# SiftScience/kafka-assigner

Hardware: NVIDIA H100
Metric: partition-replica assignments/sec (higher is better)
Workload: dtype int32

## Files before the change

kafka_assigner_b200/csrc/kassign.cu:

```cuda
#include "kassign_stage.cuh"
#include "kassign_order.cuh"
#include "kassign_json.cuh"
#include "kassign_score.cuh"
#include "kassign_waves.cuh"
#include "kassign_waves_json.cuh"

#include <algorithm>
#include <climits>
#include <cmath>
#include <cstdio>
#include <cstdlib>
#include <cstring>
#include <map>
#include <new>
#include <string>
#include <unordered_map>
#include <vector>

#include "../../include/kassign.h"

namespace {

constexpr int KA_SM_COUNT_FALLBACK = 132;
constexpr size_t KA_SMEM_BUDGET = 200 * 1024;
constexpr uint32_t KA_LUT_SMEM_MAX_RANGE = 32768;
constexpr uint32_t KA_LUT_GLOBAL_MAX_RANGE = 1u << 25;

struct DevBuf {
    void* p = nullptr;
    size_t cap = 0;
    cudaError_t reserve(size_t bytes) {
        if (bytes <= cap) return cudaSuccess;
        if (p) cudaFree(p);
        p = nullptr;
        cap = 0;
        size_t want = bytes + bytes / 8 + 256;
        cudaError_t e = cudaMalloc(&p, want);
        if (e == cudaSuccess) cap = want;
        return e;
    }
    void release() {
        if (p) cudaFree(p);
        p = nullptr;
        cap = 0;
    }
    template <typename T> T* as() const { return reinterpret_cast<T*>(p); }
};

constexpr int KA_MAX_BLOCKS = 8;
constexpr int KA_MAX_CHAIN_BLOCKS = 8;
constexpr int KA_MAX_CHAIN_EVENTS = 64;
constexpr int KA_MAX_JSON_FRAGS = 256;
constexpr int KA_MAX_CANDIDATES = 128;
static_assert(KA_MAX_CANDIDATES <= KA_JSON_MAX_SEGS, "a fleet's documents are built in one segmented JSON pass");
constexpr int64_t KA_JSON_FRAG_ROWS = 1 << 18;

struct HostPinned {
    int err_topic;
    int spin_flag;
    int4 tstatus;
};

struct Plan {
    int a_blob_bytes;
    int a_warps, a_load_bytes, a_slab_bytes, a_cnt_bytes, a_load_kind;
    int a_levels;
    int lv_owner_bytes, lv_last_bytes, lv_p_bytes;
    size_t a_smem;
    int rec_kind, rec_bytes;
    int b_gctr;
    int b_ring_log2;
    int b_threads;
    size_t b_smem;
};

struct StageDesc {
    int topic_base = 0, T = 0;
    int64_t Q = 0;
    const int32_t* d_hash = nullptr;
    const int64_t* d_part_off = nullptr;
    const int64_t* d_rep_off = nullptr;
    int P = 0, RF = 0;
    const int32_t* d_cur = nullptr;
    int desired_rf = -1, S = 1, Pmax = 0;
    int64_t capmax = 0;
    int64_t q0 = 0;
    int blk = 0;
    Plan pl;
};

struct RunScratch {
    DevBuf rec, perm, ntl, lend, loff, lvl_end, tstatus, flags;
    cudaError_t reserve(size_t rec_bytes, size_t q, size_t T, size_t nloff, bool levels, size_t nflags) {
        const struct { DevBuf* b; size_t bytes; } want[] = {
            {&rec, rec_bytes}, {&perm, levels ? q * 2 : 0}, {&lend, levels ? q * 4 : 0}, {&lvl_end, levels ? q * 4 : 0},
            {&ntl, levels ? T * 4 : 0}, {&loff, levels ? nloff * 4 : 0}, {&tstatus, T * sizeof(int4)}, {&flags, nflags * 4},
        };
        for (const auto& w : want)
            if (cudaError_t e = w.b->reserve(w.bytes)) return e;
        return cudaSuccess;
    }
    void release() {
        for (DevBuf* b : {&rec, &perm, &ntl, &lend, &loff, &lvl_end, &tstatus, &flags}) b->release();
    }
};

}

struct ka_ctx {
    int device = 0;
    int sm_count = KA_SM_COUNT_FALLBACK;
    cudaStream_t stream = nullptr;
    cudaStream_t aux = nullptr;
    cudaStream_t sb1 = nullptr;
    cudaStream_t sj = nullptr;
    KaBrokers br{};
    std::vector<int32_t> broker_id;
    DevBuf d_blob, d_glut, d_broker_id, d_ctr8;
    std::unordered_map<int32_t, std::vector<int32_t>> parked;
    int64_t launches = 0;
    DevBuf d_hash, d_part_off, d_rep_off, d_cur, d_out, d_out_len;
    RunScratch run;
    DevBuf d_json, d_names, d_name_off, d_part_id, d_json_rowlen, d_json_blocksum, d_json_state;
    DevBuf d_json_seg;
    DevBuf d_batch_tab, d_batch_ctr;
    RunScratch batch_run;
    DevBuf d_score_w, d_score_sum, d_score_brk, d_score_off;
    DevBuf d_wv_nrecv, d_wv_wave, d_wv_tmp, d_wv_rec, d_wv_cnt, d_wv_state, d_wv_log, d_wv_sum, d_wv_meta;
    DevBuf d_wv_send, d_wv_slog, d_wv_ssum;
    DevBuf d_wv_perm, d_wv_hist, d_wv_doc;
    HostPinned* h_pin = nullptr;
    unsigned long long* h_frag = nullptr;
    cudaEvent_t ev[6] = {};
    cudaEvent_t ev_pipe[KA_MAX_BLOCKS][5] = {};
    cudaEvent_t ev_chain[KA_MAX_CHAIN_EVENTS][4] = {};
    cudaEvent_t ev_in = nullptr, ev_stage[KA_MAX_BLOCKS] = {}, ev_chain_in = nullptr, ev_b1[KA_MAX_CHAIN_EVENTS] = {};
    cudaEvent_t ev_json_in[KA_MAX_JSON_FRAGS] = {}, ev_json_scan[KA_MAX_JSON_FRAGS] = {}, ev_out_done = nullptr;
    bool timing = false;
    float last_ms[8] = {};
    bool ev_valid = false;
    int last_stages = 1;
    int chain_used = 0;
    bool slot_timed[2] = {false, false};
    int32_t order_plan[8] = {};
    int32_t stage_plan[8] = {};
    bool staged = false;
    StageDesc staged_block;
    int topic_base = 0;
    bool last_was_staged = false;
    cudaStream_t last_stream = nullptr;
    bool pending_status = false;
    ka_status last{};
};

namespace {

#define KA_CUDA(call)                                                                              \
    do {                                                                                           \
        cudaError_t _e = (call);                                                                   \
        if (_e != cudaSuccess) {                                                                   \
            std::fprintf(stderr, "[kassign] CUDA error %s at %s:%d: %s\n", cudaGetErrorName(_e), __FILE__, __LINE__, \
                         cudaGetErrorString(_e));                                                  \
            return KA_ERR_CUDA;                                                                    \
        }                                                                                          \
    } while (0)

int set_status(ka_status* st, int code, int topic = -1, int part = -1, int a = 0, int b = 0) {
    if (st) {
        st->code = code;
        st->topic_index = topic;
        st->partition = part;
        st->a = a;
        st->b = b;
    }
    return code;
}

int failed(ka_status* st, int rc) {
    if (st && st->code != rc) set_status(st, rc);
    return rc;
}

inline size_t align16(size_t v) { return (v + 15) & ~size_t(15); }

template <typename F>
void for_each_event(ka_ctx* c, F f) {
    const struct { cudaEvent_t* e; size_t n; bool timed; } pools[] = {
        {c->ev, sizeof(c->ev) / sizeof(cudaEvent_t), true},
        {&c->ev_pipe[0][0], sizeof(c->ev_pipe) / sizeof(cudaEvent_t), true},
        {&c->ev_chain[0][0], sizeof(c->ev_chain) / sizeof(cudaEvent_t), true},
        {&c->ev_in, 1, false},
        {c->ev_stage, KA_MAX_BLOCKS, false},
        {&c->ev_chain_in, 1, false},
        {c->ev_b1, KA_MAX_CHAIN_EVENTS, false},
        {c->ev_json_in, KA_MAX_JSON_FRAGS, false},
        {c->ev_json_scan, KA_MAX_JSON_FRAGS, false},
        {&c->ev_out_done, 1, false},
    };
    for (const auto& p : pools)
        for (size_t i = 0; i < p.n; ++i) f(p.e[i], p.timed);
}

int park_counters(ka_ctx* c) {
    if (c->br.N == 0 || !c->d_ctr8.p) return KA_OK;
    std::vector<int32_t> h((size_t)c->br.N * KA_MAX_SLOTS);
    KA_CUDA(cudaMemcpy(h.data(), c->d_ctr8.p, h.size() * 4, cudaMemcpyDeviceToHost));
    for (int i = 0; i < c->br.N; ++i) {
        const int32_t* row = h.data() + (size_t)i * KA_MAX_SLOTS;
        bool nz = false;
        for (int r = 0; r < KA_MAX_SLOTS; ++r) nz |= row[r] != 0;
        if (nz) c->parked[c->broker_id[i]] = std::vector<int32_t>(row, row + KA_MAX_SLOTS);
        else c->parked.erase(c->broker_id[i]);
    }
    return KA_OK;
}

int check_brokers(int N, const int32_t* broker_id, const int32_t* broker_rack) {
    if (N < 0 || (N > 0 && (!broker_id || !broker_rack))) return KA_ERR_BAD_ARG;
    if (N > 65535) return KA_ERR_LIMIT;
    for (int i = 0; i < N; ++i) {
        if (i > 0 && broker_id[i] <= broker_id[i - 1]) return KA_ERR_BAD_ARG;
        if (broker_rack[i] < 0 || broker_rack[i] >= 65535) return KA_ERR_BAD_ARG;
    }
    return KA_OK;
}

struct BrokerTable {
    int lut_mode = KA_LUT_SMEM, min_id = 0, lut_off = 0;
    uint32_t range = 0;
    std::vector<uint16_t> blob, glut;
    int blob_bytes() const { return (int)(blob.size() * 2); }
    KaBrokers device(int N, const uint16_t* d_blob, const uint16_t* d_glut, const int32_t* d_broker_id) const {
        return KaBrokers{N, lut_mode, lut_off, blob_bytes(), min_id, range, d_blob, d_glut, d_broker_id};
    }
};

BrokerTable broker_table(int N, const int32_t* broker_id, const int32_t* broker_rack) {
    BrokerTable t;
    t.min_id = N > 0 ? broker_id[0] : 0;
    const uint64_t range64 = N > 0 ? (uint64_t)((int64_t)broker_id[N - 1] - (int64_t)broker_id[0]) + 1 : 0;
    const size_t npad = align16((size_t)std::max(N, 1) * 2) / 2;
    std::vector<uint16_t> rackc(std::max(N, 1), 0);
    {
        std::unordered_map<int32_t, int> seen;
        for (int i = 0; i < N; ++i) {
            auto it = seen.find(broker_rack[i]);
            if (it == seen.end()) it = seen.emplace(broker_rack[i], (int)seen.size()).first;
            rackc[i] = (uint16_t)it->second;
        }
    }
    size_t lut_elems = 0;
    if (range64 <= KA_LUT_SMEM_MAX_RANGE) {
        t.lut_mode = KA_LUT_SMEM;
        t.range = (uint32_t)range64;
        lut_elems = align16((size_t)std::max<uint64_t>(range64, 1) * 2) / 2;
    } else if (range64 <= KA_LUT_GLOBAL_MAX_RANGE) {
        t.lut_mode = KA_LUT_GLOBAL;
        t.range = (uint32_t)range64;
        t.glut.assign((size_t)range64, (uint16_t)KA_DEAD);
        for (int i = 0; i < N; ++i) t.glut[(size_t)((int64_t)broker_id[i] - t.min_id)] = (uint16_t)i;
    } else {
        t.lut_mode = KA_LUT_BSEARCH;
        t.range = 0;
    }
    t.lut_off = (int)npad;
    t.blob.assign(npad + lut_elems, (uint16_t)KA_DEAD);
    for (int i = 0; i < N; ++i) {
        t.blob[i] = rackc[i];
        if (t.lut_mode == KA_LUT_SMEM) t.blob[npad + (size_t)((int64_t)broker_id[i] - t.min_id)] = (uint16_t)i;
    }
    return t;
}

constexpr size_t KA_ORDER_SMEM_BUDGET = 226 * 1024;

int make_plan(int N, int blob_bytes, int64_t Q, int S, int Pmax, int64_t capmax, bool ragged, Plan& pl, ka_status* st) {
    if (Q >= (int64_t)1 << 31) return set_status(st, KA_ERR_LIMIT, -1, -1, INT_MAX, 0);
    pl.a_blob_bytes = blob_bytes;
    pl.a_load_kind = capmax <= 255 ? 0 : 1;
    const int lsz = pl.a_load_kind == 0 ? 1 : 2;
    pl.a_load_bytes = (int)align16((size_t)std::max(N, 1) * lsz);
    pl.a_slab_bytes = (int)align16((size_t)std::max(Pmax, 1) * S * 2);
    pl.a_cnt_bytes = (int)align16((size_t)std::max(Pmax, 1));
    pl.a_levels = (capmax > 1 || ragged) ? 1 : 0;
    if (pl.a_levels && Pmax > 32767) return set_status(st, KA_ERR_LIMIT, -1, -1, Pmax, N);
    pl.lv_owner_bytes = pl.a_levels ? (int)align16((size_t)std::max(N, 1) * 4) : 0;
    pl.lv_last_bytes = pl.a_levels ? (int)align16((size_t)std::max(N, 1) * 2) : 0;
    pl.lv_p_bytes = pl.a_levels ? (int)align16((size_t)(std::max(Pmax, 1) + 2) * 2) : 0;
    const size_t per_warp = (size_t)pl.a_load_bytes + pl.a_slab_bytes + pl.a_cnt_bytes + pl.lv_owner_bytes + pl.lv_last_bytes +
                            2 * (size_t)pl.lv_p_bytes;
    const size_t shared = 16 + (size_t)blob_bytes;
    if (shared + per_warp > KA_SMEM_BUDGET) return set_status(st, KA_ERR_LIMIT, -1, -1, Pmax, N);
    pl.a_warps = (int)std::min<size_t>(16, (KA_SMEM_BUDGET - shared) / per_warp);
    pl.a_smem = shared + per_warp * pl.a_warps;
    pl.rec_kind = S <= 3 ? 3 : (S == 4 ? 4 : 8);
    pl.rec_bytes = pl.rec_kind == 3 ? 16 : 32;
    const int cw = pl.rec_kind == 8 ? 8 : 4;
    const int max_nt = pl.rec_kind == 3 ? 1024 : (pl.rec_kind == 4 ? 512 : 256);
    const size_t ctr_bytes = pl.rec_kind == 3 ? (size_t)(std::max(N, 1) + 1) * 4 : (size_t)std::max(N, 1) * cw * 4;
    const int lg_max = pl.rec_kind == 3 ? 10 : 9, lg_min = 7;
    auto ring_bytes = [&](int l) { return ((size_t)KA_RING_STAGES << l) * pl.rec_bytes + 256; };
    int lg = lg_max;
    pl.b_gctr = 0;
    while (lg > lg_min && ctr_bytes + ring_bytes(lg) > KA_ORDER_SMEM_BUDGET) --lg;
    if (ctr_bytes + ring_bytes(lg) > KA_ORDER_SMEM_BUDGET) {
        pl.b_gctr = 1;
        lg = lg_max;
    }
    if (const char* e = std::getenv("KA_ORDER_GLOBAL_CTR")) pl.b_gctr = pl.b_gctr || std::atoi(e);
    pl.b_ring_log2 = lg;
    pl.b_smem = ring_bytes(lg) + (pl.b_gctr ? 0 : ctr_bytes);
    int64_t width = pl.a_levels ? std::min<int64_t>(Pmax, std::max<int64_t>(1, N / std::max(S, 1) / 2)) : Pmax;
    const int64_t cuts = (std::max<int64_t>(width, 1) + max_nt - 1) / max_nt;
    width = (std::max<int64_t>(width, 1) + cuts - 1) / cuts;
    int nt = (int)std::min<int64_t>(max_nt, ((width + 31) / 32) * 32);
    if (const char* e = std::getenv("KA_ORDER_THREADS")) nt = std::atoi(e);
    nt = std::max(32, std::min(max_nt, (nt / 32) * 32));
    nt = std::min(nt, (KA_RING_STAGES - 1) << lg);
    pl.b_threads = nt;
    return KA_OK;
}

template <typename K>
cudaError_t allow_smem(K kernel, size_t bytes) {
    return cudaFuncSetAttribute(kernel, cudaFuncAttributeMaxDynamicSharedMemorySize, (int)bytes);
}

struct Shape {
    int T = 0, P = 0, RF = 0, desired_rf = -1, S = 1;
    const int32_t* d_hash = nullptr;
    const int32_t* d_cur = nullptr;
    const int64_t* d_part_off = nullptr;
    const int64_t* d_rep_off = nullptr;
    int64_t Q = 0, R = 0;
    int Pmax = 0;
    int64_t capmax = 0;
};

int64_t dense_capmax(int P, int rf_t, int n) {
    return n > 0 && rf_t <= n ? ((int64_t)P * std::max(rf_t, 0) + n - 1) / n : 0;
}

Shape dense_shape(int T, int P, int RF, int desired_rf, int S, int N, const int32_t* d_hash = nullptr, const int32_t* d_cur = nullptr) {
    Shape sh{T, P, RF, desired_rf, S, d_hash, d_cur};
    sh.Q = (int64_t)T * P;
    sh.R = sh.Q * RF;
    sh.Pmax = P;
    sh.capmax = dense_capmax(P, desired_rf >= 0 ? desired_rf : RF, N);
    return sh;
}

Shape ragged_shape(int T, int64_t Q, int64_t R, int desired_rf, int S, int Pmax = 0, int64_t capmax = 0) {
    Shape sh{T, 0, 0, desired_rf, S};
    sh.Q = Q;
    sh.R = R;
    sh.Pmax = Pmax;
    sh.capmax = capmax;
    return sh;
}

int describe_block(const Shape& sh, int t0, int t1, int blk, int N, int blob_bytes, StageDesc& d, ka_status* st) {
    const bool ragged = sh.d_part_off != nullptr;
    d = StageDesc();
    d.topic_base = t0;
    d.T = t1 - t0;
    d.blk = blk;
    d.q0 = (int64_t)t0 * sh.P;
    d.Q = ragged ? sh.Q : (int64_t)d.T * sh.P;
    d.d_hash = sh.d_hash + t0;
    d.d_part_off = sh.d_part_off;
    d.d_rep_off = sh.d_rep_off;
    d.P = sh.P;
    d.RF = sh.RF;
    d.d_cur = sh.d_cur + d.q0 * sh.RF;
    d.desired_rf = sh.desired_rf;
    d.S = sh.S;
    d.Pmax = sh.Pmax;
    d.capmax = sh.capmax;
    return make_plan(N, blob_bytes, d.Q, d.S, d.Pmax, d.capmax, ragged, d.pl, st);
}

int reserve_scratch(ka_ctx* c, const StageDesc* ds, int K) {
    const StageDesc& e = ds[K - 1];
    const size_t q = (size_t)std::max<int64_t>(e.q0 + e.Q, 1);
    const size_t T = (size_t)std::max(e.topic_base + e.T, 1);
    KA_CUDA(c->run.reserve(q * ds[0].pl.rec_bytes + 256, q, T, T + K + 1, ds[0].pl.a_levels, 16));
    return KA_OK;
}

int reserve_io(ka_ctx* c, Shape& sh, bool ragged) {
    KA_CUDA(c->d_hash.reserve((size_t)std::max(sh.T, 1) * 4));
    if (ragged) {
        KA_CUDA(c->d_part_off.reserve((size_t)(sh.T + 1) * 8));
        KA_CUDA(c->d_rep_off.reserve((size_t)(sh.Q + 1) * 8));
    }
    KA_CUDA(c->d_cur.reserve((size_t)std::max<int64_t>(sh.R, 1) * 4));
    KA_CUDA(c->d_out.reserve((size_t)std::max<int64_t>(sh.Q, 1) * sh.S * 4));
    KA_CUDA(c->d_out_len.reserve((size_t)std::max<int64_t>(sh.Q, 1) * 4));
    sh.d_hash = c->d_hash.as<int32_t>();
    sh.d_cur = c->d_cur.as<int32_t>();
    if (ragged) {
        sh.d_part_off = c->d_part_off.as<int64_t>();
        sh.d_rep_off = c->d_rep_off.as<int64_t>();
    }
    return KA_OK;
}

int reset_flags(ka_ctx* c, cudaStream_t s) {
    c->h_pin->err_topic = -1;
    c->h_pin->spin_flag = -1;
    c->chain_used = 0;
    c->slot_timed[0] = c->slot_timed[1] = false;
    KA_CUDA(cudaMemsetAsync(c->run.flags.p, 0xFF, 2 * sizeof(int), s));
    return KA_OK;
}

template <typename LoadT, bool LEVELS, int SM, bool CAND>
cudaError_t launch_stage_t(ka_ctx* c, cudaStream_t s, const KaSolveParams& p, const Plan& pl, int T, int ncand, int* grid_x) {
    auto kern = ka_sticky_spread_kernel<LoadT, LEVELS, SM, CAND>;
    const int threads = pl.a_warps * 32;
    cudaError_t e = allow_smem(kern, pl.a_smem);
    if (e != cudaSuccess) return e;
    int occ = 1;
    e = cudaOccupancyMaxActiveBlocksPerMultiprocessor(&occ, kern, threads, pl.a_smem);
    if (e != cudaSuccess) return e;
    int grid = (T + pl.a_warps - 1) / pl.a_warps;
    grid = std::min(grid, std::max(1, std::max(1, occ) * c->sm_count / std::max(ncand, 1)));
    *grid_x = grid;
    kern<<<dim3(grid, std::max(ncand, 1)), threads, pl.a_smem, s>>>(p, pl.a_load_bytes, pl.a_slab_bytes, pl.a_cnt_bytes, pl.lv_owner_bytes,
                                                                 pl.lv_last_bytes, pl.lv_p_bytes);
    return cudaGetLastError();
}

template <typename LoadT, bool LEVELS, bool CAND>
cudaError_t launch_stage(ka_ctx* c, cudaStream_t s, const KaSolveParams& p, const Plan& pl, int T, int ncand, int* grid_x) {
    return p.S <= 3 ? launch_stage_t<LoadT, LEVELS, 3, CAND>(c, s, p, pl, T, ncand, grid_x)
                    : launch_stage_t<LoadT, LEVELS, 8, CAND>(c, s, p, pl, T, ncand, grid_x);
}

void reset_plans(ka_ctx* c) {
    for (int32_t& v : c->order_plan) v = 0;
    for (int32_t& v : c->stage_plan) v = 0;
}

template <bool CAND>
int launch_stage_plan(ka_ctx* c, cudaStream_t s, const KaSolveParams& p, const Plan& pl, int T, int ncand, int lut_mask) {
    cudaError_t e;
    int grid_x = 0;
    if (!pl.a_levels) e = launch_stage<uint8_t, false, CAND>(c, s, p, pl, T, ncand, &grid_x);
    else if (pl.a_load_kind == 0) e = launch_stage<uint8_t, true, CAND>(c, s, p, pl, T, ncand, &grid_x);
    else e = launch_stage<uint16_t, true, CAND>(c, s, p, pl, T, ncand, &grid_x);
    KA_CUDA(e);
    c->launches++;
    int32_t* r = c->stage_plan;
    r[0] = pl.a_load_kind == 0 ? 1 : 2;
    r[1] = pl.a_levels;
    r[2] = p.S <= 3 ? 3 : 8;
    r[3] = ncand;
    r[4] = pl.a_warps;
    r[5] = grid_x;
    r[6] = lut_mask;
    r[7]++;
    return KA_OK;
}

KaSolveParams stage_params(const StageDesc& d) {
    KaSolveParams p{};
    p.T = d.T;
    p.topic_base = d.topic_base;
    p.topic_hash = d.d_hash;
    p.part_off = d.d_part_off;
    p.P = d.P;
    p.rep_off = d.d_rep_off;
    p.RF = d.RF;
    p.cur = d.d_cur;
    p.desired_rf = d.desired_rf;
    p.S = d.S;
    p.Pmax = d.Pmax;
    p.blob_space = d.pl.a_blob_bytes;
    p.rec_kind = d.pl.rec_kind;
    p.chunk_w = d.pl.b_threads;
    return p;
}

int enq_stage(ka_ctx* c, cudaStream_t s, const StageDesc& d, cudaEvent_t a_done) {
    const Plan& pl = d.pl;
    RunScratch& r = c->run;
    if (d.T > 0) {
        KaSolveParams p = stage_params(d);
        p.br = c->br;
        p.out.rec = r.rec.as<unsigned char>() + (size_t)d.q0 * pl.rec_bytes;
        p.out.perm = pl.a_levels ? r.perm.as<uint16_t>() + d.q0 : nullptr;
        p.out.ntl = pl.a_levels ? r.ntl.as<int32_t>() + d.topic_base : nullptr;
        p.out.lend = pl.a_levels ? r.lend.as<uint32_t>() + d.q0 : nullptr;
        p.out.tstatus = r.tstatus.as<int4>();
        p.out.err_topic = r.flags.as<unsigned>();
        const int rc = launch_stage_plan<false>(c, s, p, pl, d.T, 0, 1 << c->br.lut_mode);
        if (rc != KA_OK) return rc;
    }
    if (c->timing) KA_CUDA(cudaEventRecord(a_done, s));
    if (pl.a_levels && d.T > 0) {
        int32_t* ntl = r.ntl.as<int32_t>() + d.topic_base;
        int32_t* loff = r.loff.as<int32_t>() + d.topic_base + d.blk;
        ka_level_scan_kernel<<<1, 1024, 0, s>>>(ntl, d.T, loff);
        KA_CUDA(cudaGetLastError());
        ka_level_fill_kernel<<<(d.T + 7) / 8, 256, 0, s>>>(ntl, loff, r.lend.as<uint32_t>() + d.q0, d.d_part_off, d.P, d.T, d.T, d.Q,
                                                            r.lvl_end.as<uint32_t>() + d.q0);
        KA_CUDA(cudaGetLastError());
        c->launches += 2;
    }
    return KA_OK;
}

template <int KIND, int MAXNT, bool CAND, bool GCTR, bool SINGLE, bool WARP1, bool FULL>
cudaError_t launch_order_t(cudaStream_t s, const KaOrderParams& o, const Plan& pl, int ncand) {
    auto kern = ka_order_levels_kernel<KIND, GCTR, MAXNT, SINGLE, WARP1, FULL, CAND>;
    cudaError_t e = allow_smem(kern, pl.b_smem);
    if (e != cudaSuccess) return e;
    kern<<<CAND ? ncand : 1, pl.b_threads, pl.b_smem, s>>>(o);
    return cudaGetLastError();
}

template <int KIND, int MAXNT, bool CAND = false>
cudaError_t launch_order(cudaStream_t s, const KaOrderParams& o, const Plan& pl, int* sel, int ncand = 0) {
    if constexpr (KIND > 1) {
        *sel = pl.b_gctr ? 4 : 0;
        return pl.b_gctr ? launch_order_t<KIND, MAXNT, false, true, false, false, false>(s, o, pl, ncand)
                         : launch_order_t<KIND, MAXNT, false, false, false, false, false>(s, o, pl, ncand);
    } else {
        const bool warp1 = pl.b_threads == 32;
        const bool single = !warp1 && o.uniform_width != 0 && o.uniform_width <= (uint32_t)pl.b_threads;
        const bool full = single && o.uniform_width == (uint32_t)pl.b_threads;
        *sel = (pl.b_gctr ? 4 : 0) | (warp1 ? 1 : (full ? 3 : (single ? 2 : 0)));
        switch (*sel) {
            case 0: return launch_order_t<KIND, MAXNT, CAND, false, false, false, false>(s, o, pl, ncand);
            case 1: return launch_order_t<KIND, MAXNT, CAND, false, false, true, false>(s, o, pl, ncand);
            case 2: return launch_order_t<KIND, MAXNT, CAND, false, true, false, false>(s, o, pl, ncand);
            case 3: return launch_order_t<KIND, MAXNT, CAND, false, true, false, true>(s, o, pl, ncand);
            case 4: return launch_order_t<KIND, MAXNT, CAND, true, false, false, false>(s, o, pl, ncand);
            case 5: return launch_order_t<KIND, MAXNT, CAND, true, false, true, false>(s, o, pl, ncand);
            case 6: return launch_order_t<KIND, MAXNT, CAND, true, true, false, false>(s, o, pl, ncand);
            default: return launch_order_t<KIND, MAXNT, CAND, true, true, false, true>(s, o, pl, ncand);
        }
    }
}

void note_order(ka_ctx* c, const Plan& pl, int sel, int ncand) {
    int32_t* r = c->order_plan;
    r[0] = pl.rec_kind;
    r[1] = pl.a_levels;
    r[2] = pl.b_threads;
    r[3] = pl.b_ring_log2;
    r[4] = (sel >> 2) & 1;
    r[5] = sel & 3;
    r[6]++;
    r[7] = ncand;
}

int chain_subblocks(const StageDesc& d, int blocks_in_solve) {
    if (d.d_part_off || d.pl.rec_kind != 3 || d.T < 2) return 1;
    int n = std::max(1, 8 / std::max(1, blocks_in_solve));
    n = std::min(n, std::max(1, d.T / 128));
    if (const char* e = std::getenv("KA_CHAIN_SUBBLOCKS")) n = std::max(1, std::min(std::atoi(e), d.T));
    return std::min(n, KA_MAX_CHAIN_BLOCKS);
}

struct SolveCall {
    const int32_t* h_hash = nullptr;
    const int32_t* h_cur = nullptr;
    const int64_t* h_part_off = nullptr;
    const int64_t* h_rep_off = nullptr;
    const int32_t* h_part_id = nullptr;
    int32_t* d_part_id = nullptr;
    int32_t* d_out = nullptr;
    int32_t* d_out_len = nullptr;
    int32_t* h_out = nullptr;
    int32_t* h_out_len = nullptr;
    bool json = false;
    bool stream_out = false;
    int out_copies = 0;
    int json_blocks = 0;
    int chains = 0;

    SolveCall(int32_t* out, int32_t* out_len) : d_out(out), d_out_len(out_len) {}
};

SolveCall host_call(ka_ctx* c, const int32_t* topic_hash, const int64_t* part_off, const int64_t* rep_off, const int32_t* cur_broker,
                    int32_t* out_len, int32_t* out_broker, const int32_t* part_id = nullptr) {
    SolveCall io(c->d_out.as<int32_t>(), c->d_out_len.as<int32_t>());
    io.h_hash = topic_hash;
    io.h_part_off = part_off;
    io.h_rep_off = rep_off;
    io.h_cur = cur_broker;
    io.h_part_id = part_id;
    io.d_part_id = part_id ? c->d_part_id.as<int32_t>() : nullptr;
    io.h_out = out_broker;
    io.h_out_len = out_len;
    return io;
}

struct SubBlock { int t0, t1; int64_t r0, rq; };

SubBlock sub_block(const StageDesc& d, int j, int nsub) {
    SubBlock b;
    b.t0 = (int)((int64_t)d.T * j / nsub);
    b.t1 = (int)((int64_t)d.T * (j + 1) / nsub);
    b.r0 = d.d_part_off ? 0 : (int64_t)b.t0 * d.P;
    b.rq = d.d_part_off ? d.Q : (int64_t)(b.t1 - b.t0) * d.P;
    return b;
}

KaJsonParams json_params(ka_ctx* c, const int32_t* out, const int32_t* out_len, int S, int T, const int64_t* part_off,
                         const int32_t* part_id, int64_t row0, int64_t rows, unsigned long long cap) {
    KaJsonParams p{};
    p.Q = (uint32_t)rows;
    p.row0 = (uint32_t)row0;
    p.T = T;
    p.part_off = part_off;
    p.part_id = part_id;
    p.name_off = c->d_name_off.as<int64_t>();
    p.names = c->d_names.as<char>();
    p.out = out + row0 * S;
    p.out_len = out_len + row0;
    p.S = S;
    p.rowlen = c->d_json_rowlen.as<uint32_t>() + row0;
    p.json = c->d_json.as<char>();
    p.cap = cap;
    return p;
}

KaJsonParams json_fragment(ka_ctx* c, const StageDesc& d, const SolveCall& io, int64_t row0, int64_t rows, int k) {
    KaJsonParams p = json_params(c, io.d_out, io.d_out_len, d.S, d.T, d.d_part_off, io.d_part_id, row0, rows,
                                 (unsigned long long)c->d_json.cap);
    p.blocksum = c->d_json_blocksum.as<uint32_t>() + (row0 / 256) + k;
    p.total = c->d_json_state.as<unsigned long long>();
    p.frag = p.total + 2 + 2 * k;
    return p;
}

template <bool SEG>
void enq_json_lengths(cudaStream_t s, const KaJsonParams& p, const KaJsonSegs& sg) {
    const int nblocks = (int)((p.Q + 255) / 256);
    if (nblocks > 0) ka_json_len_kernel<SEG><<<nblocks, 256, 0, s>>>(p, sg);
    ka_json_scan_kernel<<<1, 1024, 0, s>>>(p, nblocks);
}

template <typename K, typename... A>
cudaError_t enq_json_write(K kernel, unsigned grid, cudaStream_t s, const A&... args) {
    const cudaError_t e = allow_smem(kernel, KA_JSON_SMEM_BYTES + 16);
    if (e == cudaSuccess) kernel<<<grid, 256, KA_JSON_SMEM_BYTES + 16, s>>>(args...);
    return e;
}

int enq_json_rows(ka_ctx* c, cudaStream_t s_done, SolveCall& io, const StageDesc& d, const SubBlock& b, bool first, bool last) {
    const int k = io.json_blocks;
    if (k >= KA_MAX_JSON_FRAGS) return KA_ERR_LIMIT;
    KA_CUDA(cudaEventRecord(c->ev_json_in[k], s_done));
    KA_CUDA(cudaStreamWaitEvent(c->sj, c->ev_json_in[k], 0));
    KaJsonParams p = json_fragment(c, d, io, d.q0 + b.r0, b.rq, k);
    p.P = std::max(d.P, 1);
    p.topic0 = d.topic_base + b.t0;
    p.first = first;
    p.last = last;
    enq_json_lengths<false>(c->sj, p, KaJsonSegs{});
    KA_CUDA(enq_json_write(ka_json_write_kernel<false>, std::max((p.Q + 255) / 256, 1u), c->sj, p, KaJsonSegs{}));
    KA_CUDA(cudaGetLastError());
    KA_CUDA(cudaMemcpyAsync(c->h_frag + 2 * k, p.frag, 16, cudaMemcpyDeviceToHost, c->sj));
    KA_CUDA(cudaEventRecord(c->ev_json_scan[k], c->sj));
    c->launches += 3;
    io.json_blocks = k + 1;
    return KA_OK;
}

int64_t json_fragment_rows(int64_t Q) {
    const int64_t spread = (Q + KA_MAX_JSON_FRAGS - 1) / KA_MAX_JSON_FRAGS;
    return std::max(KA_JSON_FRAG_ROWS, (spread + 255) / 256 * 256);
}

int enq_json(ka_ctx* c, cudaStream_t s_done, SolveCall& io, const StageDesc& d, const SubBlock& b, bool first, bool last) {
    if (!d.d_part_off) return enq_json_rows(c, s_done, io, d, b, first, last);
    const int64_t step = json_fragment_rows(b.rq);
    int64_t r = 0;
    do {
        SubBlock f = b;
        f.r0 = b.r0 + r;
        f.rq = std::min(step, b.rq - r);
        const int rc = enq_json_rows(c, s_done, io, d, f, first && r == 0, last && r + step >= b.rq);
        if (rc != KA_OK) return rc;
        r += step;
    } while (r < b.rq);
    return KA_OK;
}

int enq_copy_out(cudaStream_t s, const SolveCall& io, int S, int64_t r0, int64_t rows) {
    KA_CUDA(cudaMemcpyAsync(io.h_out + r0 * S, io.d_out + r0 * S, (size_t)rows * S * 4, cudaMemcpyDeviceToHost, s));
    if (io.h_out_len) KA_CUDA(cudaMemcpyAsync(io.h_out_len + r0, io.d_out_len + r0, (size_t)rows * 4, cudaMemcpyDeviceToHost, s));
    return KA_OK;
}

KaOrderParams order_params(ka_ctx* c, const StageDesc& d, const SubBlock& b) {
    const Plan& pl = d.pl;
    KaOrderParams o{};
    o.N = c->br.N;
    o.S = d.S;
    o.uniform_width = pl.a_levels ? 0u : (uint32_t)d.P;
    o.chunk_end = pl.a_levels ? c->run.lvl_end.as<uint32_t>() + d.q0 : nullptr;
    o.ctr8 = c->d_ctr8.as<int32_t>();
    o.ring_log2 = pl.b_ring_log2;
    const int32_t* loff = pl.a_levels ? c->run.loff.as<int32_t>() + d.topic_base + d.blk : nullptr;
    o.Q = (uint32_t)b.rq;
    o.rec = c->run.rec.as<unsigned char>() + (size_t)(d.q0 + b.r0) * pl.rec_bytes;
    o.pos_base = (uint32_t)b.r0;
    o.chunk_lo_ptr = loff ? loff + b.t0 : nullptr;
    o.chunk_hi_ptr = loff ? loff + b.t1 : nullptr;
    return o;
}

int enq_slot_chain(ka_ctx* c, cudaStream_t s, const StageDesc& d, int slot, int j, int nsub) {
    const SubBlock b = sub_block(d, j, nsub);
    if (b.rq <= 0 || c->br.N <= 0) return KA_OK;
    const KaOrderParams o = order_params(c, d, b);
    int sel = 0;
    KA_CUDA((slot == 0 ? launch_order<0, 1024>(s, o, d.pl, &sel) : launch_order<1, 1024>(s, o, d.pl, &sel)));
    note_order(c, d.pl, sel, 0);
    c->launches++;
    return KA_OK;
}

int enq_emit_block(ka_ctx* c, cudaStream_t s, const StageDesc& d, int j, int nsub, int32_t* d_out, int32_t* d_out_len) {
    const Plan& pl = d.pl;
    const SubBlock b = sub_block(d, j, nsub);
    if (b.rq <= 0 || c->br.N <= 0) return KA_OK;
    ka_emit3_kernel<<<(unsigned)((b.rq + 255) / 256), 256, 0, s>>>(
        reinterpret_cast<const uint4*>(c->run.rec.as<unsigned char>() + (size_t)(d.q0 + b.r0) * pl.rec_bytes),
        pl.a_levels ? c->run.perm.as<uint16_t>() + d.q0 + b.r0 : nullptr, d.d_part_off, b.t1 - b.t0, d.P, c->d_broker_id.as<int32_t>(),
        (uint32_t)b.rq, d.S, d_out + (size_t)b.r0 * d.S, d_out_len ? d_out_len + b.r0 : nullptr, c->d_ctr8.as<int32_t>());
    KA_CUDA(cudaGetLastError());
    c->launches++;
    return KA_OK;
}

int enq_order_emit(ka_ctx* c, cudaStream_t s, const StageDesc& d, SolveCall& io, int blocks_in_solve) {
    const int S = d.S;
    const Plan& pl = d.pl;
    if (d.Q <= 0 || c->br.N <= 0) return io.json && d.d_part_off && d.Q == 0 ? enq_json(c, s, io, d, sub_block(d, 0, 1), true, true) : KA_OK;
    int32_t* d_out = io.d_out + d.q0 * S;
    int32_t* d_out_len = io.d_out_len ? io.d_out_len + d.q0 : nullptr;
    if (pl.rec_kind != 3) {
        const SubBlock b = sub_block(d, 0, 1);
        KaOrderParams o = order_params(c, d, b);
        o.broker_id = c->d_broker_id.as<int32_t>();
        o.out = d_out;
        o.out_len = d_out_len;
        int sel = 0;
        KA_CUDA((pl.rec_kind == 4 ? launch_order<4, 512>(s, o, pl, &sel) : launch_order<8, 256>(s, o, pl, &sel)));
        note_order(c, pl, sel, 0);
        c->launches++;
        if (io.json) return enq_json(c, s, io, d, b, d.blk == 0, d.blk == blocks_in_solve - 1);
        return KA_OK;
    }
    const int nsub = chain_subblocks(d, blocks_in_solve);
    cudaStream_t s1 = c->sb1;
    for (int j = 0; j < nsub; ++j) {
        const int e = io.chains % KA_MAX_CHAIN_EVENTS;
        if (c->timing) KA_CUDA(cudaEventRecord(c->ev_chain[e][0], s1));
        int rc = enq_slot_chain(c, s1, d, 0, j, nsub);
        if (rc != KA_OK) return rc;
        if (c->timing) KA_CUDA(cudaEventRecord(c->ev_chain[e][1], s1));
        KA_CUDA(cudaEventRecord(c->ev_b1[e], s1));
        KA_CUDA(cudaStreamWaitEvent(s, c->ev_b1[e], 0));
        if (c->timing) KA_CUDA(cudaEventRecord(c->ev_chain[e][2], s));
        if ((rc = enq_slot_chain(c, s, d, 1, j, nsub)) != KA_OK) return rc;
        if ((rc = enq_emit_block(c, s, d, j, nsub, d_out, d_out_len)) != KA_OK) return rc;
        if (c->timing) KA_CUDA(cudaEventRecord(c->ev_chain[e][3], s));
        const SubBlock b = sub_block(d, j, nsub);
        if (io.stream_out) {
            cudaStream_t so = s;
            if (io.out_copies < KA_MAX_CHAIN_EVENTS) {
                KA_CUDA(cudaEventRecord(c->ev_json_in[io.out_copies], s));
                KA_CUDA(cudaStreamWaitEvent(c->sj, c->ev_json_in[io.out_copies], 0));
                io.out_copies++;
                so = c->sj;
            }
            if ((rc = enq_copy_out(so, io, S, d.q0 + b.r0, b.rq)) != KA_OK) return rc;
        }
        if (io.json) {
            if ((rc = enq_json(c, s, io, d, b, d.blk == 0 && j == 0, d.blk == blocks_in_solve - 1 && j == nsub - 1)) != KA_OK)
                return rc;
        }
        c->chain_used = std::min(++io.chains, KA_MAX_CHAIN_EVENTS);
    }
    return KA_OK;
}

int chain_fork(ka_ctx* c, cudaStream_t s) {
    KA_CUDA(cudaEventRecord(c->ev_chain_in, s));
    KA_CUDA(cudaStreamWaitEvent(c->sb1, c->ev_chain_in, 0));
    return KA_OK;
}

int enq_solve_end(ka_ctx* c, cudaStream_t s) {
    KA_CUDA(cudaMemcpyAsync(&c->h_pin->err_topic, c->run.flags.p, 2 * sizeof(int), cudaMemcpyDeviceToHost, s));
    if (c->timing) {
        KA_CUDA(cudaEventRecord(c->ev[5], s));
        c->ev_valid = true;
    }
    return KA_OK;
}

int pipeline_stages(int T, int64_t Q) {
    int k = Q >= 262144 ? std::min(4, T / 2048) : 1;
    if (const char* e = std::getenv("KA_PIPELINE_STAGES")) k = std::atoi(e);
    return std::max(1, std::min(k, std::min(KA_MAX_BLOCKS, std::max(T, 1))));
}

int enq_inputs(cudaStream_t s, const SolveCall& io, const StageDesc& d, int64_t ncur) {
    auto h2d = [&](const void* dst, const void* src, size_t bytes) {
        return cudaMemcpyAsync(const_cast<void*>(dst), src, bytes, cudaMemcpyHostToDevice, s);
    };
    if (io.h_hash && d.T > 0) KA_CUDA(h2d(d.d_hash, io.h_hash + d.topic_base, (size_t)d.T * 4));
    if (io.h_part_off && d.T > 0) KA_CUDA(h2d(d.d_part_off, io.h_part_off, (size_t)(d.T + 1) * 8));
    if (io.h_rep_off && d.Q > 0) KA_CUDA(h2d(d.d_rep_off, io.h_rep_off, (size_t)(d.Q + 1) * 8));
    if (io.h_part_id && d.Q > 0) KA_CUDA(h2d(io.d_part_id, io.h_part_id, (size_t)d.Q * 4));
    if (io.h_cur && ncur > 0) KA_CUDA(h2d(d.d_cur, io.h_cur + d.q0 * d.RF, (size_t)ncur * 4));
    return KA_OK;
}

int run_solve(ka_ctx* c, cudaStream_t s, const Shape& sh, SolveCall& io, ka_status* st) {
    c->staged = false;
    c->last_was_staged = false;
    reset_plans(c);
    const bool ragged = sh.d_part_off != nullptr;
    const int T = sh.T;
    const int K = ragged ? 1 : pipeline_stages(T, (int64_t)T * sh.P);
    const bool host_io = (io.h_cur != nullptr || io.h_out != nullptr) && K >= 3;
    const int wsum = host_io ? 2 * (K - 1) : K;
    auto bound = [&](int k) { return k <= 0 ? 0 : (k >= K ? T : (int)((int64_t)T * (host_io ? 2 * k - 1 : k) / wsum)); };
    StageDesc ds[KA_MAX_BLOCKS];
    int rc;
    for (int k = 0; k < K; ++k)
        if ((rc = describe_block(sh, bound(k), bound(k + 1), k, c->br.N, c->br.blob_bytes, ds[k], st)) != KA_OK) return rc;
    if ((rc = reserve_scratch(c, ds, K)) != KA_OK) return rc;
    c->last_stages = K;
    if (c->timing) KA_CUDA(cudaEventRecord(c->ev[0], s));
    if (K == 1) {
        const StageDesc& d = ds[0];
        if ((rc = enq_inputs(s, io, d, ragged ? sh.R : d.Q * d.RF)) != KA_OK) return rc;
        if ((rc = reset_flags(c, s)) != KA_OK) return rc;
        if (c->timing) KA_CUDA(cudaEventRecord(c->ev[1], s));
        if ((rc = enq_stage(c, s, d, c->ev[2])) != KA_OK) return rc;
        if (c->timing) KA_CUDA(cudaEventRecord(c->ev[3], s));
        if ((rc = chain_fork(c, s)) != KA_OK) return rc;
        if ((rc = enq_order_emit(c, s, d, io, 1)) != KA_OK) return rc;
        if (c->timing) KA_CUDA(cudaEventRecord(c->ev[4], s));
        if (io.h_out && d.Q > 0 && c->br.N > 0 && (rc = enq_copy_out(s, io, d.S, 0, d.Q)) != KA_OK) return rc;
    } else {
        cudaStream_t aux = c->aux;
        io.stream_out = io.h_out && ds[0].pl.rec_kind == 3 && !io.json;
        KA_CUDA(cudaEventRecord(c->ev_in, s));
        if (io.stream_out) KA_CUDA(cudaStreamWaitEvent(c->sj, c->ev_in, 0));
        KA_CUDA(cudaStreamWaitEvent(aux, c->ev_in, 0));
        if ((rc = reset_flags(c, aux)) != KA_OK) return rc;
        for (int k = 0; k < K; ++k) {
            const StageDesc& d = ds[k];
            if ((rc = enq_inputs(aux, io, d, d.Q * d.RF)) != KA_OK) return rc;
            if (c->timing) KA_CUDA(cudaEventRecord(c->ev_pipe[k][0], aux));
            if ((rc = enq_stage(c, aux, d, c->ev_pipe[k][1])) != KA_OK) return rc;
            if (c->timing) KA_CUDA(cudaEventRecord(c->ev_pipe[k][2], aux));
            KA_CUDA(cudaEventRecord(c->ev_stage[k], aux));
            KA_CUDA(cudaStreamWaitEvent(s, c->ev_stage[k], 0));
            KA_CUDA(cudaStreamWaitEvent(c->sb1, c->ev_stage[k], 0));
            if (k == 0) KA_CUDA(cudaStreamWaitEvent(c->sb1, c->ev_in, 0));
            if (c->timing) KA_CUDA(cudaEventRecord(c->ev_pipe[k][3], s));
            if ((rc = enq_order_emit(c, s, d, io, K)) != KA_OK) return rc;
            if (c->timing) KA_CUDA(cudaEventRecord(c->ev_pipe[k][4], s));
            if (io.h_out && !io.stream_out && d.Q > 0 && c->br.N > 0 && (rc = enq_copy_out(s, io, d.S, d.q0, d.Q)) != KA_OK) return rc;
        }
        if (io.stream_out) {
            KA_CUDA(cudaEventRecord(c->ev_out_done, c->sj));
            KA_CUDA(cudaStreamWaitEvent(s, c->ev_out_done, 0));
        }
    }
    return enq_solve_end(c, s);
}

ka_status topic_status(int t, const int4& ts, const int32_t* part_id, const int64_t* part_off) {
    ka_status r;
    set_status(&r, ts.x, t, ts.y >= 0 && part_id && part_off ? part_id[part_off[t] + ts.y] : ts.y, ts.z, ts.w);
    return r;
}

int finish_status(ka_ctx* c, cudaStream_t s, ka_status* st, const int32_t* part_id = nullptr, const int64_t* part_off = nullptr) {
    KA_CUDA(cudaStreamSynchronize(s));
    c->pending_status = false;
    ka_status r{};
    set_status(&r, KA_OK);
    if (c->h_pin->err_topic != -1) {
        const int t = c->h_pin->err_topic;
        KA_CUDA(cudaMemcpy(&c->h_pin->tstatus, c->run.tstatus.as<int4>() + t, sizeof(int4), cudaMemcpyDeviceToHost));
        r = topic_status(t, c->h_pin->tstatus, part_id, part_off);
        r.topic_index += c->last_was_staged ? c->topic_base : 0;
    }
    if (c->timing && c->ev_valid) {
        for (int i = 0; i < 8; ++i) c->last_ms[i] = 0.f;
        cudaEventElapsedTime(&c->last_ms[5], c->ev[0], c->ev[5]);
        if (c->last_stages <= 1) {
            cudaEventElapsedTime(&c->last_ms[3], c->ev[0], c->ev[1]);
            cudaEventElapsedTime(&c->last_ms[0], c->ev[1], c->ev[2]);
            cudaEventElapsedTime(&c->last_ms[1], c->ev[2], c->ev[3]);
            cudaEventElapsedTime(&c->last_ms[7], c->ev[3], c->ev[4]);
            cudaEventElapsedTime(&c->last_ms[4], c->ev[4], c->ev[5]);
        } else {
            for (int k = 0; k < c->last_stages; ++k) {
                float a = 0.f, t = 0.f, b = 0.f;
                cudaEventElapsedTime(&a, c->ev_pipe[k][0], c->ev_pipe[k][1]);
                cudaEventElapsedTime(&t, c->ev_pipe[k][1], c->ev_pipe[k][2]);
                cudaEventElapsedTime(&b, c->ev_pipe[k][3], c->ev_pipe[k][4]);
                c->last_ms[0] += a;
                c->last_ms[1] += t;
                c->last_ms[7] += b;
            }
        }
        if (c->chain_used > 0) {
            for (int e = 0; e < c->chain_used; ++e) {
                float b1 = 0.f, b2 = 0.f;
                cudaEventElapsedTime(&b1, c->ev_chain[e][0], c->ev_chain[e][1]);
                cudaEventElapsedTime(&b2, c->ev_chain[e][2], c->ev_chain[e][3]);
                c->last_ms[2] += b1;
                c->last_ms[6] += b2;
            }
        } else if (c->slot_timed[0] || c->slot_timed[1]) {
            if (c->slot_timed[0]) cudaEventElapsedTime(&c->last_ms[2], c->ev_chain[0][0], c->ev_chain[0][1]);
            if (c->slot_timed[1]) cudaEventElapsedTime(&c->last_ms[6], c->ev_chain[1][0], c->ev_chain[1][1]);
        } else {
            c->last_ms[2] = c->last_ms[7];
        }
    }
    c->last = r;
    if (st) *st = r;
    return r.code;
}

int enter(ka_ctx* c, bool collect) {
    KA_CUDA(cudaSetDevice(c->device));
    if (collect && c->pending_status) finish_status(c, c->last_stream, nullptr);
    return KA_OK;
}

int finish(ka_ctx* c, cudaStream_t s, ka_status* st, bool sync, const int32_t* part_id = nullptr, const int64_t* part_off = nullptr) {
    c->last_stream = s;
    c->pending_status = true;
    return st || sync ? finish_status(c, s, st, part_id, part_off) : KA_OK;
}

int fail_members(ka_status* st, int K, int rc) {
    for (int k = 0; k < K; ++k) set_status(st + k, rc);
    return rc;
}

int abort_batch(ka_ctx* c, cudaStream_t s, ka_status* st, int K, int rc) {
    cudaStreamSynchronize(c->sb1);
    cudaStreamSynchronize(s);
    return fail_members(st, K, rc);
}

int batch_args(ka_ctx* c, int K, int out_stride, ka_status* st) {
    if (!st || K < 0) return KA_ERR_BAD_ARG;
    for (int k = 0; k < K; ++k) set_status(st + k, KA_OK);
    if (!c) return fail_members(st, K, KA_ERR_NO_DEVICE);
    if (K > KA_MAX_CANDIDATES || out_stride > 3) return fail_members(st, K, KA_ERR_LIMIT);
    if (out_stride < 1) return fail_members(st, K, KA_ERR_BAD_ARG);
    return KA_OK;
}

int check_tables(int K, const int32_t* cand_off, const int32_t* broker_id, const int32_t* broker_rack) {
    if (!cand_off || cand_off[0] != 0) return KA_ERR_BAD_ARG;
    for (int k = 0; k < K; ++k) {
        const int n = cand_off[k + 1] - cand_off[k];
        if (cand_off[k + 1] < cand_off[k] || (n > 0 && (!broker_id || !broker_rack))) return KA_ERR_BAD_ARG;
        const int rc = n > 0 ? check_brokers(n, broker_id + cand_off[k], broker_rack + cand_off[k]) : KA_OK;
        if (rc != KA_OK) return rc;
    }
    return KA_OK;
}

struct BatchMember {
    int tab = 0;
    int t0 = 0, T = 0;
    int64_t row0 = 0, Q = 0;
    int desired_rf = -1;
    int64_t rec0 = 0;
    int64_t topic0 = 0;
    int n = 0, blob_bytes = 0;
    int Pmax = 0;
    int64_t capmax = 0;
    int S = 1;
};

struct Batch {
    int K = 0;
    const int32_t* cand_off = nullptr;
    const int32_t* broker_id = nullptr;
    std::vector<BrokerTable> tabs;
    std::vector<BatchMember> m;
    int64_t recs = 0;
    int topics = 0;
    int fill_T = 0;
    int64_t fill_rows = 0;
    int64_t out_rows = 0;
    int nmax = 0, blob_max = 0, Pmax = 0, Tmax = 0;
    int64_t capmax = 0, Qmax = 0;

    void add(const BatchMember& mb) {
        m.push_back(mb);
        nmax = std::max(nmax, mb.n);
        blob_max = std::max(blob_max, mb.blob_bytes);
        Pmax = std::max(Pmax, mb.Pmax);
        capmax = std::max(capmax, mb.capmax);
        Tmax = std::max(Tmax, mb.T);
        Qmax = std::max(Qmax, mb.Q);
    }
};

int batch_tables(ka_ctx* c, int K, const int32_t* cand_off, const int32_t* broker_id, const int32_t* broker_rack, int64_t recs,
                 Batch& b, ka_status* st) {
    if (recs >= ((int64_t)1 << 31)) return fail_members(st, K, KA_ERR_LIMIT);
    const int rc = enter(c, true);
    if (rc != KA_OK) return fail_members(st, K, rc);
    reset_plans(c);
    b.K = K;
    b.cand_off = cand_off;
    b.broker_id = broker_id;
    b.tabs.resize(K);
    for (int k = 0; k < K; ++k)
        b.tabs[k] = broker_table(cand_off[k + 1] - cand_off[k], broker_id + cand_off[k], broker_rack + cand_off[k]);
    return KA_OK;
}

void add_candidates(Batch& b, int T, int64_t Q, int Pmax, int desired_rf, const std::vector<int64_t>& capmax) {
    const int64_t q = std::max<int64_t>(Q, 1);
    for (int k = 0; k < b.K; ++k)
        b.add(BatchMember{k, 0, T, 0, Q, desired_rf, (int64_t)k * q, (int64_t)k * T, b.cand_off[k + 1] - b.cand_off[k],
                          b.tabs[k].blob_bytes(), Pmax, capmax[k]});
    b.recs = (int64_t)b.K * q;
    b.topics = b.K * T;
    b.fill_T = T;
    b.fill_rows = Q;
    b.out_rows = Q;
}

void add_clusters(Batch& b, int T, int64_t Q, const std::vector<BatchMember>& passed, ka_status* st) {
    for (BatchMember mb : passed) {
        mb.blob_bytes = b.tabs[mb.tab].blob_bytes();
        Plan own;
        if (make_plan(mb.n, mb.blob_bytes, mb.Q, mb.S, mb.Pmax, mb.capmax, true, own, st + mb.tab) == KA_OK) b.add(mb);
    }
    b.recs = std::max<int64_t>(Q, 1);
    b.topics = T;
    b.fill_T = std::max(T, 1);
    b.out_rows = 0;
    if (b.Tmax == 0) b.m.clear();
}

int plan_batch(Shape sh, const Batch& b, StageDesc& d, ka_status* st) {
    sh.Pmax = b.Pmax;
    sh.capmax = b.capmax;
    const int rc = describe_block(sh, 0, sh.T, 0, b.nmax, b.blob_max, d, st);
    for (int k = 1; k < b.K && rc != KA_OK; ++k) st[k] = st[0];
    return rc;
}

int finish_batch(ka_ctx* c, cudaStream_t s, const Batch& b, ka_status* st, const int32_t* part_id = nullptr,
                 const int64_t* part_off = nullptr) {
    const int K = b.K, M = (int)b.m.size();
    if (cudaStreamSynchronize(s) != cudaSuccess) return fail_members(st, K, KA_ERR_CUDA);
    std::vector<unsigned> err(std::max(M, 1));
    if (M > 0 && cudaMemcpy(err.data(), c->batch_run.flags.p, (size_t)M * 4, cudaMemcpyDeviceToHost) != cudaSuccess)
        return fail_members(st, K, KA_ERR_CUDA);
    for (int k = 0; k < M; ++k) {
        if (err[k] == 0xFFFFFFFFu) continue;
        const BatchMember& mb = b.m[k];
        const int t = (int)err[k] - mb.t0;
        int4 ts;
        if (cudaMemcpy(&ts, c->batch_run.tstatus.as<int4>() + mb.topic0 + t, sizeof(int4), cudaMemcpyDeviceToHost) != cudaSuccess)
            return fail_members(st, K, KA_ERR_CUDA);
        st[mb.tab] = topic_status(mb.t0 + t, ts, part_id, part_off);
        st[mb.tab].topic_index = t;
    }
    for (int k = 0; k < K; ++k)
        if (st[k].code != KA_OK) return st[k].code;
    return KA_OK;
}

template <typename F>
// ... 1354 lines not shown
```

Measured before the change: 2.837 billion.

## Move emit, copy-out and JSON stages onto a third stream for overlap

The emit kernel, streamed output copy and JSON encoding for each chain sub-block now run on a separate stream (sj), gated by a new per-sub-block event recorded after slot-1 on the main stream. Slot 0 and slot 1 of the next sub-block can therefore proceed while the previous sub-block's emit and output work is in flight, forming a three-stage pipeline. The main stream joins on the last emit event at the end. This adds cross-stream event traffic and relies on the ordering of the sj stream being correct for JSON state that was previously serialized on the main stream.

```diff
diff --git a/kafka_assigner_b200/csrc/kassign.cu b/kafka_assigner_b200/csrc/kassign.cu
--- a/kafka_assigner_b200/csrc/kassign.cu
+++ b/kafka_assigner_b200/csrc/kassign.cu
@@ -135,6 +135,7 @@
     cudaEvent_t ev_pipe[KA_MAX_BLOCKS][5] = {};
     cudaEvent_t ev_chain[KA_MAX_CHAIN_EVENTS][4] = {};
     cudaEvent_t ev_in = nullptr, ev_stage[KA_MAX_BLOCKS] = {}, ev_chain_in = nullptr, ev_b1[KA_MAX_CHAIN_EVENTS] = {};
+    cudaEvent_t ev_b2[KA_MAX_CHAIN_EVENTS] = {}, ev_emit = nullptr;
     cudaEvent_t ev_json_in[KA_MAX_JSON_FRAGS] = {}, ev_json_scan[KA_MAX_JSON_FRAGS] = {}, ev_out_done = nullptr;
     bool timing = false;
     float last_ms[8] = {};
@@ -193,6 +194,8 @@
         {c->ev_stage, KA_MAX_BLOCKS, false},
         {&c->ev_chain_in, 1, false},
         {c->ev_b1, KA_MAX_CHAIN_EVENTS, false},
+        {c->ev_b2, KA_MAX_CHAIN_EVENTS, false},
+        {&c->ev_emit, 1, false},
         {c->ev_json_in, KA_MAX_JSON_FRAGS, false},
         {c->ev_json_scan, KA_MAX_JSON_FRAGS, false},
         {&c->ev_out_done, 1, false},
@@ -578,7 +581,6 @@
     int32_t* h_out_len = nullptr;
     bool json = false;
     bool stream_out = false;
-    int out_copies = 0;
     int json_blocks = 0;
     int chains = 0;
 
@@ -760,36 +762,29 @@
         return KA_OK;
     }
     const int nsub = chain_subblocks(d, blocks_in_solve);
-    cudaStream_t s1 = c->sb1;
+    cudaStream_t s1 = c->sb1, se = c->sj;
     for (int j = 0; j < nsub; ++j) {
         const int e = io.chains % KA_MAX_CHAIN_EVENTS;
+        const cudaEvent_t done0 = c->timing ? c->ev_chain[e][1] : c->ev_b1[e];
         if (c->timing) KA_CUDA(cudaEventRecord(c->ev_chain[e][0], s1));
         int rc = enq_slot_chain(c, s1, d, 0, j, nsub);
         if (rc != KA_OK) return rc;
-        if (c->timing) KA_CUDA(cudaEventRecord(c->ev_chain[e][1], s1));
-        KA_CUDA(cudaEventRecord(c->ev_b1[e], s1));
-        KA_CUDA(cudaStreamWaitEvent(s, c->ev_b1[e], 0));
+        KA_CUDA(cudaEventRecord(done0, s1));
+        KA_CUDA(cudaStreamWaitEvent(s, done0, 0));
         if (c->timing) KA_CUDA(cudaEventRecord(c->ev_chain[e][2], s));
         if ((rc = enq_slot_chain(c, s, d, 1, j, nsub)) != KA_OK) return rc;
-        if ((rc = enq_emit_block(c, s, d, j, nsub, d_out, d_out_len)) != KA_OK) return rc;
-        if (c->timing) KA_CUDA(cudaEventRecord(c->ev_chain[e][3], s));
+        KA_CUDA(cudaEventRecord(c->ev_b2[e], s));
+        KA_CUDA(cudaStreamWaitEvent(se, c->ev_b2[e], 0));
+        if ((rc = enq_emit_block(c, se, d, j, nsub, d_out, d_out_len)) != KA_OK) return rc;
+        KA_CUDA(cudaEventRecord(c->ev_emit, se));
+        if (c->timing) KA_CUDA(cudaEventRecord(c->ev_chain[e][3], se));
         const SubBlock b = sub_block(d, j, nsub);
-        if (io.stream_out) {
-            cudaStream_t so = s;
-            if (io.out_copies < KA_MAX_CHAIN_EVENTS) {
-                KA_CUDA(cudaEventRecord(c->ev_json_in[io.out_copies], s));
-                KA_CUDA(cudaStreamWaitEvent(c->sj, c->ev_json_in[io.out_copies], 0));
-                io.out_copies++;
-                so = c->sj;
-            }
-            if ((rc = enq_copy_out(so, io, S, d.q0 + b.r0, b.rq)) != KA_OK) return rc;
-        }
-        if (io.json) {
-            if ((rc = enq_json(c, s, io, d, b, d.blk == 0 && j == 0, d.blk == blocks_in_solve - 1 && j == nsub - 1)) != KA_OK)
-                return rc;
-        }
+        if (io.stream_out && (rc = enq_copy_out(se, io, S, d.q0 + b.r0, b.rq)) != KA_OK) return rc;
+        if (io.json && (rc = enq_json(c, se, io, d, b, d.blk == 0 && j == 0, d.blk == blocks_in_solve - 1 && j == nsub - 1)) != KA_OK)
+            return rc;
         c->chain_used = std::min(++io.chains, KA_MAX_CHAIN_EVENTS);
     }
+    KA_CUDA(cudaStreamWaitEvent(s, c->ev_emit, 0));
     return KA_OK;
 }
 
```

Result: faster. 2.942 billion, median of 6 (+3.7%).
